# sangminwoo/SVOL

Measured on AMD Instinct MI355X. Metric: frames/sec (fwd+matcher+bwd), T=32·P=196·d=256, higher is better.
Workload: dtype bf16

## Files before the change

### svol_amd/blocks.py

```python
from __future__ import annotations

import ctypes
import math
import os
import weakref

import torch

from . import _lib, layers, ops, params, wgrad

ENABLED = os.environ.get('SVOL_NO_BLOCKS') is None
GATE_SCORES_FUSE = os.environ.get('SVOL_GATE_SCORES_FUSE') is not None
VH, QS, QC = 0, 1, 2
_F32, _BF16 = 0, 1
_ESZ = {torch.float32: 4, torch.bfloat16: 2, torch.float16: 2}
_SLOTS = {}


def _slots(block):
    m = _SLOTS.get(block)
    if m is None:
        names = _lib.lib().svol_block_slot_names(block).decode().rstrip(',').split(',')
        m = _SLOTS[block] = {n: i for i, n in enumerate(names)}
    return m
# ... 283 lines not shown
class _DqPrezero:
    __slots__ = ('bufs', 'side', 'ev_prep', 'clean_ev', 'clean', 'nxt')

    def __init__(self, dev, wsb):
        self.bufs = [torch.empty((_align(wsb, 1 << 20),), dtype=torch.uint8, device=dev) for _ in range(2)]
        self.side = torch.cuda.Stream(device=dev)
        self.ev_prep = torch.cuda.Event()
        self.clean_ev = [torch.cuda.Event(), torch.cuda.Event()]
        for e_ in [self.ev_prep] + self.clean_ev:
            e_.record()
        self.clean = [False, False]
        self.nxt = 0

    def bind(self, tbl):
        i = self.nxt
        tbl.set('ATTN_WS', self.bufs[i].data_ptr())
        tbl.set('EV_CLEAN_IN', self.clean_ev[i].cuda_event if self.clean[i] else None)
        tbl.set('EV_PREP', self.ev_prep.cuda_event)
        tbl.set('ATTN_WS_NEXT', self.bufs[1 - i].data_ptr())
        tbl.set('ZERO_STREAM', self.side.cuda_stream)
        tbl.set('EV_CLEAN_OUT', self.clean_ev[1 - i].cuda_event)
        self.clean[i] = False

    def advance(self, tbl):
        i = self.nxt
        self.clean[1 - i] = True
        self.nxt = 1 - i
        for n_ in ('EV_CLEAN_IN', 'EV_PREP', 'ATTN_WS_NEXT', 'ZERO_STREAM', 'EV_CLEAN_OUT'):
            tbl.set(n_, None)


def _dq_prezero(dev, B, H, L, dh, dt, wsb):
    if not DQ_PREZERO or dt == torch.float32 or torch.cuda.is_current_stream_capturing():
        return None
    key = (dev, ops._stream(), B, H, L, dh, dt, wsb)
    st = _DQ_PREZERO.get(key)
    if st is None:
        img = _lib.lib().svol_attn_bwd_sp_image_bytes(B, H, L, L, dh, wsb, ops._DT[dt])
        st = _DQ_PREZERO[key] = _DqPrezero(dev, wsb) if img > 0 else False
    return st or None


def _vh_fwd_layout(B, L, D, H, F, e):
    M = B * L
    return [('Y1', M * D * e), ('Y1POS', M * D * e), ('A', M * 4), ('MEAN1', M * 4), ('RSTD1', M * 4), ('GATE_WS', B * H * (L + 2) * 4),
            ('QKV', M * 3 * D * e), ('O', M * D * e), ('LSE', B * H * L * 4), ('S2', M * D * 4), ('Y2', M * D * e), ('MEAN2', M * 4),
            ('RSTD2', M * 4), ('PRE', M * F * e), ('HID', M * F * e), ('S3', M * D * 4), ('MEAN3', M * 4), ('RSTD3', M * 4),
            ('M32', M * D * 4), ('M', M * D * e), ('MPOS', M * D * e)]


def _vh_bwd_layout(B, L, D, H, F, e):
    M = B * L
    return [('DS32_3', M * D * 4), ('DS3', M * D * e), ('DPRE', M * F * e), ('DY2', M * D * e), ('DS32_2', M * D * 4), ('G2D', M * D * e),
            ('DO', M * D * e), ('DQKV', M * 3 * D * e), ('DELTA', 3 * B * H * L * 4), ('DXQP', M * D * e), ('DXQ', M * D * e),
            ('GATE_WS2', (B * L + B * H) * 4), ('DX32', M * D * 4)]


def _attn_events(tbl, ev):
    tbl.set('EV_A0', ev[0].cuda_event if ev else None)
    tbl.set('EV_A1', ev[1].cuda_event if ev else None)


class VideoHalfFn(torch.autograd.Function):

    @staticmethod
    def forward(ctx, pl, x32, pos, u, u_next, sc_in, *params):
        B, L, D = x32.shape
        layer = pl.layer()
        H, F = layer.nhead, layer.mlp1.fc1.weight.shape[0]
        dt = pl.dt
        e = _ESZ[dt]
        dev = x32.device
        M = B * L
        x2, pos2, u = _c(x32.reshape(M, D)), _c(pos.reshape(M, D)), _c(u)
        assert x2.dtype == torch.float32 and pos2.dtype == dt and u.dtype == torch.float32
        wsb = ops.attn_ws_bytes(dt, B, H, L, L, D // H)
        lay = _open(ctx, pl, VH, (B, L, D, H, F, dt), _dims(B, L, 0, D, H, F, dt, dt, wsb), len(params), dev,
                    lambda: _vh_fwd_layout(B, L, D, H, F, e),
                    lambda: [('Y1_32', M * D * 4), ('Y2_32', M * D * 4), ('ATTN_WS', max(wsb, 16))], X32=x2, POS=pos2, U=u)
        tbl = ctx.tbl
        if sc_in is not None:
            assert sc_in.dtype == torch.float32 and sc_in.numel() == B * H * (L + 2) and sc_in.is_contiguous()
            tbl.set('GATE_WS', sc_in.data_ptr())
            tbl.set('GATE_PRE', sc_in.data_ptr())
        if u_next is not None:
            u_next = u_next.contiguous()
            assert u_next.dtype == torch.float32 and u_next.shape == u.shape and L % 4 == 0
            sc_next = torch.empty((B * H * (L + 2),), dtype=torch.float32, device=dev)
            tbl.set('U_NEXT', u_next.data_ptr())
            tbl.set('GATE_WS_NEXT', sc_next.data_ptr())
        else:
            sc_next = torch.empty((0,), dtype=torch.float32, device=dev)
        ctx.big = wgrad.attn_forward(B * H * L * L)
        _attn_events(tbl, _maybe_events('attn_fwd', (B, H, L, L, D // H)))
        _call('svol_video_half_fwd', ctx)
        _attn_events(tbl, None)
        tbl.set('U_NEXT', None)
        tbl.set('GATE_WS_NEXT', None)
        ctx.shape = (B, L, D, H, F)
        ctx.sc_in = sc_in
        ctx.save_for_backward(x2, pos2, u)
        ctx.mark_non_differentiable(sc_next)
        return (lay.view(ctx.arena, 'M32', torch.float32, (B, L, D)), lay.view(ctx.arena, 'M', dt, (B, L, D)),
                lay.view(ctx.arena, 'MPOS', dt, (B, L, D)), sc_next)

    @staticmethod
    def backward(ctx, dm32, dm, dmpos, _dsc=None):
# ... 49 lines not shown

class QuerySelfFn(torch.autograd.Function):

    @staticmethod
    def forward(ctx, pl, o32, o, opos, qpos, *params):
        B, N, D = o.shape
        H, qdt = pl.layer().nhead, pl.qdt
        e, R = _ESZ[qdt], B * N
        o32_, o_, opos_, qpos_ = _c(o32), _c(o), _c(opos), _c(qpos)
        assert o32_.dtype == torch.float32 and o_.dtype == qdt and opos_.dtype == qdt and qpos_.dtype == qdt
        wsb = ops.attn_ws_bytes(qdt, B, H, N, N, D // H)
        lay = _open(ctx, pl, QS, (B, N, D, H, qdt), _dims(B, 0, N, D, H, 0, qdt, qdt, wsb), len(params), o.device,
                    lambda: [('QKV', R * 3 * D * e), ('OA', R * D * e), ('LSE', B * H * N * 4), ('S4', R * D * 4), ('MEAN4', R * 4),
                             ('RSTD4', R * 4), ('Y32', R * D * 4), ('Y', R * D * e), ('YPOS', R * D * e)],
                    lambda: [('ATTN_WS', max(wsb, 16))], O32=o32_, O=o_, OPOS=opos_, QPOS=qpos_)
        _call('svol_query_self_fwd', ctx)
        ctx.shape = (B, N, D, H)
        ctx.save_for_backward(o32_, o_, opos_, qpos)
        return (lay.view(ctx.arena, 'Y32', torch.float32, (B, N, D)), lay.view(ctx.arena, 'Y', qdt, (B, N, D)),
                lay.view(ctx.arena, 'YPOS', qdt, (B, N, D)))

    @staticmethod
    def backward(ctx, dy32, dy, dypos):
        if dy32 is None and dy is None and dypos is None:
            return _no_grads(ctx, 5)
        B, N, D, H = ctx.shape
        o32_, o_, opos_, qpos = ctx.saved_tensors
        qdt = ctx.pl.qdt
        e, R = _ESZ[qdt], B * N
        gq = _qpos_target(ctx, qpos, ctx.needs_input_grad[4], N, D)
        lay, tmp, bufs, gs = _open_bwd(ctx, o_.device, lambda: [('G', R * D * e), ('DOA', R * D * e), ('DQKV', R * 3 * D * e),
                                                               ('DELTA', 3 * B * H * N * 4), ('DO32', R * D * 4), ('DXQ', R * D * e),
                                                               ('DXQP', R * D * e)], DY32=dy32, DY=dy, DYPOS=dypos)
        _call('svol_query_self_bwd', ctx)
        pg = _close_bwd(ctx, 'svol_query_self_wgrad', bufs, [ctx.arena, tmp, o_, opos_], 5)
        v = lambda n_, dt_: lay.view(tmp, n_, dt_, (B, N, D))
        return (None, v('DO32', torch.float32), v('DXQ', qdt), v('DXQP', qdt), _qpos_grad(gq, qdt)) + pg


def query_self(layer, out, qpos, dt, qdt):
    pl = plan(layer, QS, dt, qdt)
    o32, o, opos = out
    return QuerySelfFn.apply(pl, o32, o, opos, qpos, *pl.inputs(o32, o, opos))


def _qc_fwd_layout(B, N, L, D, H, F, e, qe):
    R, M = B * N, B * L
    return [('Q', R * D * qe), ('QC', R * D * e), ('KV', M * 2 * D * e), ('OA', R * D * e), ('OAQ', R * D * qe), ('LSE', B * H * N * 4),
            ('S5', R * D * 4), ('Y5_32', R * D * 4), ('Y5', R * D * qe), ('MEAN5', R * 4), ('RSTD5', R * 4), ('PRE', R * F * qe),
            ('HID', R * F * qe), ('S6', R * D * 4), ('MEAN6', R * 4), ('RSTD6', R * 4), ('Y32', R * D * 4), ('Y', R * D * qe),
            ('YPOS', R * D * qe)]


def _qc_bwd_layout(B, N, L, D, H, F, e, qe):
    R, M = B * N, B * L
    return [('DS32_6', R * D * 4), ('DS6', R * D * qe), ('DPRE', R * F * qe), ('DY5', R * D * qe), ('G5D', R * D * qe), ('DOAQ', R * D * qe),
            ('DOA', R * D * e), ('DQC', R * D * e), ('DQ', R * D * qe), ('DKV', M * 2 * D * e), ('DELTA', 3 * B * H * N * 4),
            ('DO32', R * D * 4), ('DXQP', R * D * qe), ('DMPOS', M * D * e), ('DMV', M * D * e)]


class QueryCrossFn(torch.autograd.Function):

    @staticmethod
    def forward(ctx, pl, o32, o, opos, mv, mpos, kbias, qpos, *params):
        B, N, D = o.shape
        L = mv.shape[1]
        layer = pl.layer()
        H, F = layer.nhead, layer.mlp2.fc1.weight.shape[0]
        dt, qdt = pl.dt, pl.qdt
        e, qe = _ESZ[dt], _ESZ[qdt]
        o32_, o_, opos_, mv_, mpos_, kb_, qpos_ = _c(o32), _c(o), _c(opos), _c(mv), _c(mpos), _c(kbias), _c(qpos)
        assert o32_.dtype == torch.float32 and o_.dtype == qdt and opos_.dtype == qdt and qpos_.dtype == qdt
        assert mv_.dtype == dt and mpos_.dtype == dt and kb_.dtype == torch.float32
        wsb = ops.attn_ws_bytes(dt, B, H, N, L, D // H)
        lay = _open(ctx, pl, QC, (B, N, L, D, H, F, dt, qdt), _dims(B, L, N, D, H, F, dt, qdt, wsb), len(params), o.device,
                    lambda: _qc_fwd_layout(B, N, L, D, H, F, e, qe), lambda: [('ATTN_WS', max(wsb, 16))],
                    O32=o32_, O=o_, OPOS=opos_, MV=mv_, MPOS=mpos_, KBIAS=kb_, QPOS=qpos_)
        _call('svol_query_cross_fwd', ctx)
        ctx.shape = (B, N, L, D, H, F)
        ctx.save_for_backward(o32_, o_, opos_, mv_, mpos_, kb_, qpos)
        return (lay.view(ctx.arena, 'Y32', torch.float32, (B, N, D)), lay.view(ctx.arena, 'Y', qdt, (B, N, D)),
                lay.view(ctx.arena, 'YPOS', qdt, (B, N, D)))

    @staticmethod
    def backward(ctx, dy32, dy, dypos):
        if dy32 is None and dy is None and dypos is None:
            return _no_grads(ctx, 8)
        B, N, L, D, H, F = ctx.shape
        o32_, o_, opos_, mv_, mpos_, kb_, qpos = ctx.saved_tensors
        dt, qdt = ctx.pl.dt, ctx.pl.qdt
        gq = _qpos_target(ctx, qpos, ctx.needs_input_grad[7], N, D)
        lay, tmp, bufs, gs = _open_bwd(ctx, o_.device, lambda: _qc_bwd_layout(B, N, L, D, H, F, _ESZ[dt], _ESZ[qdt]),
                                       DY32=dy32, DY=dy, DYPOS=dypos)
        _call('svol_query_cross_bwd', ctx)
        pg = _close_bwd(ctx, 'svol_query_cross_wgrad', bufs, [ctx.arena, tmp, opos_, mv_, mpos_], 8)
        vq = lambda n_, dt_: lay.view(tmp, n_, dt_, (B, N, D))
        vm = lambda n_: lay.view(tmp, n_, dt, (B, L, D))
        return (None, vq('DO32', torch.float32), None, vq('DXQP', qdt), vm('DMV'), vm('DMPOS'), None, _qpos_grad(gq, qdt)) + pg


def query_cross(layer, out, mv, mpos, kbias, qpos, dt, qdt):
    pl = plan(layer, QC, dt, qdt)
    o32, o, opos = out
    return QueryCrossFn.apply(pl, o32, o, opos, mv, mpos, kbias, qpos, *pl.inputs(o32, opos, mv, mpos))


def trace_dump() -> str:
    buf = ctypes.create_string_buffer(1 << 20)
    _lib.check(_lib.lib().svol_block_trace_dump(buf, len(buf)), 'svol_block_trace_dump')
    return buf.value.decode()
```

### svol_amd/csrc/blocks.hip

```cpp
#include <math.h>
#include <stdio.h>
#include <stdlib.h>
#include <string.h>

#include <map>
#include <mutex>
#include <string>
#include <vector>

#include "common.h"

namespace {

const bool kTrace = getenv("SVOL_BLOCK_TRACE") != nullptr;
struct TraceRec { const char* prog; const char* site; hipEvent_t e0, e1; };
std::mutex g_trace_mu;
std::vector<TraceRec> g_trace_log;
struct Trace {
    const char* prog;
    hipStream_t s;
    hipEvent_t last = nullptr;
    Trace* prev;
    static thread_local Trace* cur;
    Trace(const char* prog_, void* s_) : prog(prog_), s(static_cast<hipStream_t>(s_)), prev(cur) {
// ... 151 lines not shown
        RUN(nt(P(Y1), D, at(P(W_IN), 2 * D * D, dt), D, at(P(QKV), 2 * D, dt), 3 * D, f32(P(B_IN)) + 2 * D, nullptr, M, D, D, dt, s));
    record(P(EV_A0), s);
    RUN(svol_attn_fwd(P(QKV), 3 * D, at(P(QKV), D, dt), 3 * D, at(P(QKV), 2 * D, dt), 3 * D, P(O), D, f32(P(LSE)), nullptr, d.B, d.H, d.L,
                      d.L, dh, attn_scale(dh), attn_premul(dh, dt), P(ATTN_WS), d.ws_bytes, dt, s));
    record(P(EV_A1), s);
    RUN(nt_res(P(O), D, P(W_O), D, P(S2), P(B_O), P(Y1_32), M, D, D, dt, s));
    RUN(svol_layernorm_fwd(P(S2), xf, f32(P(G2)), f32(P(BT2)), f32(P(Y2_32)), P(Y2), nullptr, nullptr, 0, f32(P(MEAN2)), f32(P(RSTD2)), M,
                           D, 0.f, 0, nullptr, dt, s));
    RUN(svol_gemm_nt(P(Y2), D, nullptr, 0, P(W_FC1), D, P(HID), F, f32(P(B_FC1)), nullptr, SVOL_ACT_GELU_D, P(PRE), F, nullptr, 0, 0, M, F, D, dt, s));
    RUN(nt_res(P(HID), F, P(W_FC2), F, P(S3), P(B_FC2), P(Y2_32), M, D, F, dt, s));
    if (P(U_NEXT) && P(GATE_WS_NEXT))
        RUN(svol_layernorm_gate_scores_fwd(f32(P(S3)), f32(P(G3)), f32(P(BT3)), f32(P(M32)), P(M), P(MPOS), P(POS), f32(P(MEAN3)),
                                           f32(P(RSTD3)), f32(P(U_NEXT)), f32(P(GATE_WS_NEXT)), d.B, d.L, D, d.H, dt, s));
    else
        RUN(svol_layernorm_fwd(P(S3), xf, f32(P(G3)), f32(P(BT3)), f32(P(M32)), P(M), P(MPOS), P(POS), M, f32(P(MEAN3)), f32(P(RSTD3)), M, D,
                               0.f, 0, nullptr, dt, s));
    return SVOL_OK;
}

int svol_video_half_bwd(const int64_t* dims, void* const* p, int phase, void* s) {
    if (!dims || !p || phase < 0 || phase > 2) return SVOL_E_INVALID;
    Trace tr_(phase == 2 ? "video_half_bwd.2" : "video_half_bwd.1", s);
    const Dims d(dims);
    if (!d.ok() || d.L <= 0 || d.F <= 0) return SVOL_E_INVALID;
    const int64_t M = d.B * d.L, D = d.D, F = d.F, dh = D / d.H;
    const int dt = d.dt, xf = dt != SVOL_F32;
    if (phase != 2) {
        RUN(svol_layernorm_bwd(f32(P(DM32)), P(DM), P(DMPOS), P(S3), xf, f32(P(G3)), f32(P(MEAN3)), f32(P(RSTD3)), f32(P(DS32_3)), P(DS3),
                               f32(P(DG3)), f32(P(DBT3)), f32(P(DB_FC2)), M, D, 0.f, 0, nullptr, dt, s));
        RUN(svol_gemm_nt_dact(P(DS3), D, P(W_FC2_T), D, P(DPRE), F, P(PRE), F, SVOL_ACT_GELU_D, f32(P(DB_FC1)), M, F, D, dt, s));
        RUN(nt(P(DPRE), F, P(W_FC1_T), F, P(DY2), D, nullptr, nullptr, M, D, F, dt, s));
        RUN(svol_layernorm_bwd(f32(P(DS32_3)), P(DY2), nullptr, P(S2), xf, f32(P(G2)), f32(P(MEAN2)), f32(P(RSTD2)), f32(P(DS32_2)), P(G2D),
                               f32(P(DG2)), f32(P(DBT2)), f32(P(DB_O)), M, D, 0.f, 0, nullptr, dt, s));
        RUN(nt(P(G2D), D, P(W_O_T), D, P(DO), D, nullptr, nullptr, M, D, D, dt, s));
    }
    if (phase != 1) {
        int aflags = 0;
        if (P(EV_CLEAN_IN)) {
            if (hipStreamWaitEvent(static_cast<hipStream_t>(s), static_cast<hipEvent_t>(P(EV_CLEAN_IN)), 0) != hipSuccess) return SVOL_E_LAUNCH;
            aflags = SVOL_ATTN_DQ_PREZEROED;
        }
        record(P(EV_A0), s);
        RUN(svol_attn_bwd_ex(P(QKV), 3 * D, at(P(QKV), D, dt), 3 * D, at(P(QKV), 2 * D, dt), 3 * D, P(O), D, P(DO), D, f32(P(LSE)),
                             f32(P(DELTA)), nullptr, P(DQKV), 3 * D, at(P(DQKV), D, dt), 3 * D, at(P(DQKV), 2 * D, dt), 3 * D, d.B, d.H, d.L,
                             d.L, dh, attn_scale(dh), attn_premul(dh, dt), P(ATTN_WS), d.ws_bytes, dt, aflags, P(EV_PREP), s));
        record(P(EV_A1), s);
        if (P(ATTN_WS_NEXT) && P(ZERO_STREAM) && P(EV_PREP) && P(EV_CLEAN_OUT)) {
            hipStream_t zs = static_cast<hipStream_t>(P(ZERO_STREAM));
            if (hipStreamWaitEvent(zs, static_cast<hipEvent_t>(P(EV_PREP)), 0) != hipSuccess) return SVOL_E_LAUNCH;
            const int zrc = svol_attn_bwd_zero_ws(P(ATTN_WS_NEXT), d.ws_bytes, d.B, d.H, d.L, d.L, dh, dt, zs);
            if (zrc) return zrc;
            record(P(EV_CLEAN_OUT), zs);
        }
        RUN(nt(P(DQKV), 3 * D, P(W_IN_T), 3 * D, P(DXQP), D, nullptr, nullptr, M, D, 2 * D, dt, s));
        RUN(nt(at(P(DQKV), 2 * D, dt), 3 * D, at(P(W_IN_T), 2 * D, dt), 3 * D, P(DXQ), D, nullptr, nullptr, M, D, D, dt, s));
        RUN(svol_gate_bwd(f32(P(DS32_2)), P(DXQ), P(DXQP), f32(P(X32)), P(POS), f32(P(U)), f32(P(G1)), f32(P(A)), f32(P(MEAN1)),
                          f32(P(RSTD1)), f32(P(GATE_WS)), f32(P(GATE_WS2)), f32(P(DX32)), f32(P(DU)), f32(P(DG1)), f32(P(DBT1)), d.B, d.L,
                          D, d.H, dt, s));
    }
    return SVOL_OK;
}

int svol_video_half_wgrad_part(const int64_t* dims, void* const* p, int part, void* s) {
    if (!dims || !p || part < 0 || part > 2) return SVOL_E_INVALID;
    Trace tr_(part == 1 ? "video_half_wgrad.1" : part == 2 ? "video_half_wgrad.2" : "video_half_wgrad", s);
    const Dims d(dims);
    if (!d.ok()) return SVOL_E_INVALID;
    const int64_t M = d.B * d.L, D = d.D, F = d.F;
    const int dt = d.dt;
    const svol_tn_problem pr[5] = {
        {P(DS3), D, P(HID), F, f32(P(DW_FC2)), F, nullptr, M, D, F},
        {P(DPRE), F, P(Y2), D, f32(P(DW_FC1)), D, nullptr, M, F, D},
        {P(G2D), D, P(O), D, f32(P(DW_O)), D, nullptr, M, D, D},
        {P(DQKV), 3 * D, P(Y1POS), D, f32(P(DW_IN)), D, f32(P(DB_IN)), M, 2 * D, D},
        {at(P(DQKV), 2 * D, dt), 3 * D, P(Y1), D, f32(P(DW_IN)) + 2 * D * D, D, f32(P(DB_IN)) + 2 * D, M, D, D}};
    if (part == 1) RUN(svol_gemm_tn_grouped(pr, 3, dt, s));
    else if (part == 2) RUN(svol_gemm_tn_grouped(pr + 3, 2, dt, s));
    else RUN(svol_gemm_tn_grouped(pr, 5, dt, s));
    return SVOL_OK;
}

int svol_video_half_wgrad(const int64_t* dims, void* const* p, void* s) { return svol_video_half_wgrad_part(dims, p, 0, s); }
#undef P

int svol_query_self_fwd(const int64_t* dims, void* const* p, void* s) {
    if (!dims || !p) return SVOL_E_INVALID;
    Trace tr_("query_self_fwd", s);
    const Dims d(dims);
    if (!d.ok() || d.N <= 0) return SVOL_E_INVALID;
    const int64_t R = d.B * d.N, D = d.D, dh = D / d.H;
    const int qdt = d.qdt, xf = qdt != SVOL_F32;
#define P(n) p[SVOL_QS_##n]
    RUN(nt(P(OPOS), D, P(W_IN), D, P(QKV), 3 * D, P(B_IN), P(QSCALE), R, 2 * D, D, qdt, s));
    if (P(WV_HILO))
        RUN(svol_gemm_nt_split(P(O), D, P(WV_HILO), 2 * D, at(P(QKV), 2 * D, qdt), 3 * D, f32(P(B_IN)) + 2 * D, R, D, D, s));
    else
        RUN(nt(P(O), D, at(P(W_IN), 2 * D * D, qdt), D, at(P(QKV), 2 * D, qdt), 3 * D, f32(P(B_IN)) + 2 * D, nullptr, R, D, D, qdt, s));
    RUN(svol_attn_fwd(P(QKV), 3 * D, at(P(QKV), D, qdt), 3 * D, at(P(QKV), 2 * D, qdt), 3 * D, P(OA), D, f32(P(LSE)), nullptr, d.B, d.H,
                      d.N, d.N, dh, attn_scale(dh), attn_premul(dh, qdt), P(ATTN_WS), d.ws_bytes, qdt, s));
    RUN(nt_res(P(OA), D, P(W_O), D, P(S4), P(B_O), P(O32), R, D, D, qdt, s));
    RUN(svol_layernorm_fwd(P(S4), xf, f32(P(G4)), f32(P(BT4)), f32(P(Y32)), P(Y), P(YPOS), P(QPOS), d.N, f32(P(MEAN4)), f32(P(RSTD4)), R, D,
                           0.f, 0, nullptr, qdt, s));
    return SVOL_OK;
}

int svol_query_self_bwd(const int64_t* dims, void* const* p, void* s) {
    if (!dims || !p) return SVOL_E_INVALID;
    Trace tr_("query_self_bwd", s);
    const Dims d(dims);
// ... 41 lines not shown
    if (mixed) {
        RUN(nt(P(OPOS), D, P(W_INQ), D, P(Q), D, P(B_IN), P(QSCALE), R, D, D, qdt, s));
        RUN(svol_cast(P(Q), qdt, P(QC), dt, R * D, s));
    } else {
        RUN(nt(P(OPOS), D, P(W_KV), D, P(QC), D, P(B_IN), P(QSCALE), R, D, D, dt, s));
    }
    RUN(nt(P(MPOS), D, at(P(W_KV), D * D, dt), D, P(KV), 2 * D, f32(P(B_IN)) + D, nullptr, M, D, D, dt, s));
    if (P(WV_HILO))
        RUN(svol_gemm_nt_split(P(MV), D, P(WV_HILO), 2 * D, at(P(KV), D, dt), 2 * D, f32(P(B_IN)) + 2 * D, M, D, D, s));
    else
        RUN(nt(P(MV), D, at(P(W_KV), 2 * D * D, dt), D, at(P(KV), D, dt), 2 * D, f32(P(B_IN)) + 2 * D, nullptr, M, D, D, dt, s));
    RUN(svol_attn_fwd(P(QC), D, P(KV), 2 * D, at(P(KV), D, dt), 2 * D, P(OA), D, f32(P(LSE)), f32(P(KBIAS)), d.B, d.H, d.N, d.L, dh,
                      attn_scale(dh), attn_premul(dh, dt), P(ATTN_WS), d.ws_bytes, dt, s));
    const void* oq = P(OA);
    if (mixed) {
        RUN(svol_cast(P(OA), dt, P(OAQ), qdt, R * D, s));
        oq = P(OAQ);
    }
    RUN(nt_res(oq, D, P(W_O), D, P(S5), P(B_O), P(O32), R, D, D, qdt, s));
    RUN(svol_layernorm_fwd(P(S5), xf, f32(P(G5)), f32(P(BT5)), f32(P(Y5_32)), P(Y5), nullptr, nullptr, 0, f32(P(MEAN5)), f32(P(RSTD5)), R,
                           D, 0.f, 0, nullptr, qdt, s));
    RUN(svol_gemm_nt(P(Y5), D, nullptr, 0, P(W_FC1), D, P(HID), F, f32(P(B_FC1)), nullptr, SVOL_ACT_GELU, P(PRE), F, nullptr, 0, 0, R, F, D,
                     qdt, s));
    RUN(nt_res(P(HID), F, P(W_FC2), F, P(S6), P(B_FC2), P(Y5_32), R, D, F, qdt, s));
    RUN(svol_layernorm_fwd(P(S6), xf, f32(P(G6)), f32(P(BT6)), f32(P(Y32)), P(Y), P(YPOS), P(QPOS), d.N, f32(P(MEAN6)), f32(P(RSTD6)), R, D,
                           0.f, 0, nullptr, qdt, s));
    return SVOL_OK;
}

int svol_query_cross_bwd(const int64_t* dims, void* const* p, void* s) {
    if (!dims || !p) return SVOL_E_INVALID;
    Trace tr_("query_cross_bwd", s);
    const Dims d(dims);
    if (!d.ok() || d.N <= 0 || d.L <= 0 || d.F <= 0) return SVOL_E_INVALID;
    const int64_t R = d.B * d.N, M = d.B * d.L, D = d.D, F = d.F, dh = D / d.H;
    const int dt = d.dt, qdt = d.qdt, xf = qdt != SVOL_F32;
    const bool mixed = qdt != dt;
    RUN(svol_layernorm_bwd(f32(P(DY32)), P(DY), P(DYPOS), P(S6), xf, f32(P(G6)), f32(P(MEAN6)), f32(P(RSTD6)), f32(P(DS32_6)), P(DS6),
                           f32(P(DG6)), f32(P(DBT6)), f32(P(DB_FC2)), R, D, 0.f, 0, nullptr, qdt, s));
    if (P(DQPOS) && P(DYPOS)) RUN(svol_colsum(P(DYPOS), d.N * D, f32(P(DQPOS)), d.B, d.N * D, qdt, s));
    RUN(svol_gemm_nt_dact(P(DS6), D, P(W_FC2_T), D, P(DPRE), F, P(PRE), F, SVOL_ACT_GELU, f32(P(DB_FC1)), R, F, D, qdt, s));
    RUN(nt(P(DPRE), F, P(W_FC1_T), F, P(DY5), D, nullptr, nullptr, R, D, F, qdt, s));
    RUN(svol_layernorm_bwd(f32(P(DS32_6)), P(DY5), nullptr, P(S5), xf, f32(P(G5)), f32(P(MEAN5)), f32(P(RSTD5)), f32(P(DO32)), P(G5D),
                           f32(P(DG5)), f32(P(DBT5)), f32(P(DB_O)), R, D, 0.f, 0, nullptr, qdt, s));
    RUN(nt(P(G5D), D, P(W_O_T), D, P(DOAQ), D, nullptr, nullptr, R, D, D, qdt, s));
    const void* d_o = P(DOAQ);
    if (mixed) {
        RUN(svol_cast(P(DOAQ), qdt, P(DOA), dt, R * D, s));
        d_o = P(DOA);
    }
    RUN(svol_attn_bwd(P(QC), D, P(KV), 2 * D, at(P(KV), D, dt), 2 * D, P(OA), D, d_o, D, f32(P(LSE)), f32(P(DELTA)), f32(P(KBIAS)), P(DQC), D,
                      P(DKV), 2 * D, at(P(DKV), D, dt), 2 * D, d.B, d.H, d.N, d.L, dh, attn_scale(dh), attn_premul(dh, dt), P(ATTN_WS),
                      d.ws_bytes, dt, s));
    RUN(nt(P(DKV), 2 * D, at(P(W_KV_T), D, dt), 3 * D, P(DMPOS), D, nullptr, nullptr, M, D, D, dt, s));
    RUN(nt(at(P(DKV), D, dt), 2 * D, at(P(W_KV_T), 2 * D, dt), 3 * D, P(DMV), D, nullptr, nullptr, M, D, D, dt, s));
    const void* dq = P(DQC);
    if (mixed) {
        RUN(svol_cast(P(DQC), dt, P(DQ), qdt, R * D, s));
        dq = P(DQ);
    }
    RUN(nt(dq, D, mixed ? P(W_INQ_T) : P(W_KV_T), 3 * D, P(DXQP), D, nullptr, nullptr, R, D, D, qdt, s));
    return SVOL_OK;
}

int svol_query_cross_wgrad(const int64_t* dims, void* const* p, void* s) {
    if (!dims || !p) return SVOL_E_INVALID;
    Trace tr_("query_cross_wgrad", s);
    const Dims d(dims);
    if (!d.ok()) return SVOL_E_INVALID;
    const int64_t R = d.B * d.N, M = d.B * d.L, D = d.D, F = d.F;
    const int dt = d.dt, qdt = d.qdt;
    const bool mixed = qdt != dt;
    const svol_tn_problem pv[2] = {
        {P(DKV), 2 * D, P(MPOS), D, f32(P(DW_IN)) + D * D, D, f32(P(DB_IN)) + D, M, D, D},
        {at(P(DKV), D, dt), 2 * D, P(MV), D, f32(P(DW_IN)) + 2 * D * D, D, f32(P(DB_IN)) + 2 * D, M, D, D}};
    RUN(svol_gemm_tn_grouped(pv, 2, dt, s));
    const svol_tn_problem pq[4] = {
        {P(DS6), D, P(HID), F, f32(P(DW_FC2)), F, nullptr, R, D, F},
        {P(DPRE), F, P(Y5), D, f32(P(DW_FC1)), D, nullptr, R, F, D},
        {P(G5D), D, mixed ? P(OAQ) : P(OA), D, f32(P(DW_O)), D, nullptr, R, D, D},
        {mixed ? P(DQ) : P(DQC), D, P(OPOS), D, f32(P(DW_IN)), D, f32(P(DB_IN)), R, D, D}};
    RUN(svol_gemm_tn_grouped(pq, 4, qdt, s));
    return SVOL_OK;
#undef P
}

}
```

### svol_amd/csrc/gemm_n256_bf16.hip

```cpp
#include <type_traits>

#include "gemm_call.h"

namespace {

struct N256Args {
    const h16_t* A; const h16_t* W; void* C;
    const float* bias; const float* res;
    int64_t lda, ldw, ldc, ldr;
    int M, K, act, nrt;
    int kwt;
};

typedef __attribute__((address_space(3))) void* lds_void_ptr;

constexpr int BM = 128, BN = 256, BK = 32, STG = 3;
constexpr int A_ST = BM * BK * 2;
constexpr int W_ST = BN * BK * 2;
constexpr int SLOT = A_ST + W_ST;

__device__ __forceinline__ int slot32(int row, int ch) { return ch ^ ((0x78 >> (2 * ((row >> 2) & 3))) & 3); }
__device__ __forceinline__ int wcol(int nt, int i) { return (nt >> 1) * 32 + (i >> 2) * 8 + (nt & 1) * 4 + (i & 3); }

template <int N> __device__ __forceinline__ void n256_wait_vm() { asm volatile("s_waitcnt vmcnt(%0)" ::"n"(N) : "memory"); }

template <int OFF>
__device__ __forceinline__ void read_frags(uint4 (&af)[4], uint4 (&wf)[8], const unsigned (&aa)[4], const unsigned (&wa)[8]) {
    asm volatile(
        "ds_read_b128 %0, %12 offset:%c24\n\t"
        "ds_read_b128 %1, %13 offset:%c24\n\t"
        "ds_read_b128 %2, %14 offset:%c24\n\t"
        "ds_read_b128 %3, %15 offset:%c24\n\t"
        "ds_read_b128 %4, %16 offset:%c25\n\t"
        "ds_read_b128 %5, %17 offset:%c25\n\t"
        "ds_read_b128 %6, %18 offset:%c25\n\t"
        "ds_read_b128 %7, %19 offset:%c25\n\t"
        "ds_read_b128 %8, %20 offset:%c25\n\t"
        "ds_read_b128 %9, %21 offset:%c25\n\t"
        "ds_read_b128 %10, %22 offset:%c25\n\t"
        "ds_read_b128 %11, %23 offset:%c25\n\t"
        "s_waitcnt lgkmcnt(0)"
        : "=&v"(af[0]), "=&v"(af[1]), "=&v"(af[2]), "=&v"(af[3]), "=&v"(wf[0]), "=&v"(wf[1]), "=&v"(wf[2]), "=&v"(wf[3]),
          "=&v"(wf[4]), "=&v"(wf[5]), "=&v"(wf[6]), "=&v"(wf[7])
        : "v"(aa[0]), "v"(aa[1]), "v"(aa[2]), "v"(aa[3]), "v"(wa[0]), "v"(wa[1]), "v"(wa[2]), "v"(wa[3]), "v"(wa[4]), "v"(wa[5]),
          "v"(wa[6]), "v"(wa[7]), "n"(OFF), "n"(OFF + A_ST)
        : "memory");
}

template <bool OUT_F32>
__device__ __forceinline__ void gemm_n256_body(const N256Args& p) {
    __shared__ __attribute__((aligned(1024))) char smem[STG * SLOT];
    const int tid = threadIdx.x, lane = tid & 63;
    const int wave = __builtin_amdgcn_readfirstlane(tid >> 6);
    const int wm = wave >> 1, wn = wave & 1;
    const int fr = lane & 15, fq = lane >> 4;
    const int rt = blockIdx.x % p.nrt, cg = blockIdx.x / p.nrt;
    const int bm = rt * BM;
    if (bm >= p.M) return;
    const int rows = min(BM, p.M - bm);
    const int bn = cg * BN;

    const __amdgpu_buffer_rsrc_t rA = __builtin_amdgcn_make_buffer_rsrc(
        (void*)(p.A + (int64_t)bm * p.lda), 0, (int)((((int64_t)rows - 1) * p.lda + p.kwt * BK) * 2), 0x00020000);
    const __amdgpu_buffer_rsrc_t rW =
        __builtin_amdgcn_make_buffer_rsrc((void*)(p.W + (int64_t)bn * p.ldw), 0, (int)((((int64_t)BN - 1) * p.ldw + p.K) * 2), 0x00020000);
    int voffA[2], voffW[4];
#pragma unroll
    for (int j = 0; j < 2; ++j) {
        const int row = (wave * 2 + j) * 16 + (lane >> 2);
        voffA[j] = (int)(((int64_t)row * p.lda + slot32(row, lane & 3) * 8) * 2);
    }
#pragma unroll
    for (int j = 0; j < 4; ++j) {
        const int rho = (wave * 4 + j) * 16 + (lane >> 2);
        const int n = (rho >> 7) * 128 + wcol((rho & 127) >> 4, rho & 15);
        voffW[j] = (int)(((int64_t)n * p.ldw + slot32(rho, lane & 3) * 8) * 2);
    }
    auto issue = [&](int slot, int kt) {
        char* sl = smem + slot * SLOT;
        const int so = kt * BK * 2;
        const int soA = (kt >= p.kwt ? kt - p.kwt : kt) * BK * 2;
#pragma unroll
        for (int j = 0; j < 2; ++j)
            __builtin_amdgcn_raw_ptr_buffer_load_lds(rA, (lds_void_ptr)(sl + (wave * 2 + j) * 1024), 16, voffA[j], soA, 0, 0);
#pragma unroll
        for (int j = 0; j < 4; ++j)
            __builtin_amdgcn_raw_ptr_buffer_load_lds(rW, (lds_void_ptr)(sl + A_ST + (wave * 4 + j) * 1024), 16, voffW[j], so, 0, 0);
    };

    const unsigned lds0 = (unsigned)(size_t)(lds_void_ptr)smem;
    unsigned aa[4], wa[8];
#pragma unroll
    for (int mt = 0; mt < 4; ++mt) {
        const int row = wm * 64 + mt * 16 + fr;
        aa[mt] = lds0 + (unsigned)(row * 64 + (slot32(row, fq) << 4));
    }
#pragma unroll
    for (int nt = 0; nt < 8; ++nt) {
        const int rho = wn * 128 + nt * 16 + fr;
        wa[nt] = lds0 + (unsigned)(rho * 64 + (slot32(rho, fq) << 4));
    }

    f32x4 acc[8][4];
#pragma unroll
    for (int i = 0; i < 8; ++i)
#pragma unroll
        for (int j = 0; j < 4; ++j) acc[i][j] = f32x4{0.f, 0.f, 0.f, 0.f};

    const int nk = p.K / BK;
    issue(0, 0);
    if (nk > 1) issue(1, 1);
    auto step = [&](auto slot_tag, int kt) {
        constexpr int S = decltype(slot_tag)::value;
        if (kt + 1 < nk) n256_wait_vm<6>(); else n256_wait_vm<0>();
        __builtin_amdgcn_s_barrier();
        if (kt + 2 < nk) issue((S + 2) % STG, kt + 2);
        uint4 af[4], wf[8];
        read_frags<S * SLOT>(af, wf, aa, wa);
#pragma unroll
        for (int nt = 0; nt < 8; ++nt)
#pragma unroll
            for (int mt = 0; mt < 4; ++mt)
                acc[nt][mt] = SVOL_MFMA_16x16x32_H16(__builtin_bit_cast(h16x8, wf[nt]),
                                                                      __builtin_bit_cast(h16x8, af[mt]), acc[nt][mt], 0, 0, 0);
    };
    int kt = 0;
    for (; kt + 3 <= nk; kt += 3) {
        step(std::integral_constant<int, 0>{}, kt);
        step(std::integral_constant<int, 1>{}, kt + 1);
        step(std::integral_constant<int, 2>{}, kt + 2);
    }
    if (kt < nk) step(std::integral_constant<int, 0>{}, kt++);
    if (kt < nk) step(std::integral_constant<int, 1>{}, kt++);

#pragma unroll
    for (int mt = 0; mt < 4; ++mt) {
        const int m = bm + wm * 64 + mt * 16 + fr;
        if (m >= p.M) continue;
#pragma unroll
        for (int pr = 0; pr < 4; ++pr) {
            const int n0 = bn + wn * 128 + pr * 32 + fq * 8;
            float v[8];
#pragma unroll
            for (int e = 0; e < 8; ++e) v[e] = acc[2 * pr + (e >> 2)][mt][e & 3];
            if (p.bias) {
#pragma unroll
                for (int e = 0; e < 8; ++e) v[e] += p.bias[n0 + e];
            }
            if constexpr (OUT_F32) {
                float* C = reinterpret_cast<float*>(p.C) + (int64_t)m * p.ldc + n0;
                if (p.res) {
                    const float* R = p.res + (int64_t)m * p.ldr + n0;
                    const f32x4 r0 = *reinterpret_cast<const f32x4*>(R), r1 = *reinterpret_cast<const f32x4*>(R + 4);
#pragma unroll
                    for (int e = 0; e < 4; ++e) { v[e] += r0[e]; v[4 + e] += r1[e]; }
                }
                *reinterpret_cast<f32x4*>(C) = f32x4{v[0], v[1], v[2], v[3]};
                *reinterpret_cast<f32x4*>(C + 4) = f32x4{v[4], v[5], v[6], v[7]};
            } else {
                if (act_is_gelu(p.act)) {
#pragma unroll
                    for (int e = 0; e < 8; ++e) v[e] = gelu_fast(v[e]);
                }
                if (p.act == SVOL_ACT_RELU) {
#pragma unroll
                    for (int e = 0; e < 8; ++e) v[e] = fmaxf(v[e], 0.f);
                }
                h16x8 o;
#pragma unroll
                for (int e = 0; e < 8; ++e) o[e] = (h16_t)v[e];
                *reinterpret_cast<h16x8*>(reinterpret_cast<h16_t*>(p.C) + (int64_t)m * p.ldc + n0) = o;
            }
        }
    }
}

__global__ __launch_bounds__(256, 2) void gemm_n256_bf16_f32(N256Args p) { gemm_n256_body<true>(p); }
__global__ __launch_bounds__(256, 2) void gemm_n256_bf16_b16(N256Args p) { gemm_n256_body<false>(p); }

}

static int n256_plan(const GemmCall& c, N256Args& p, dim3& grid) {
    const int64_t M = c.M, N = c.N, K = c.K;
    if (N % BN || K % BK || K < 512 || M < 4096) return SVOL_E_UNSUPPORTED;
    if (c.epi != 0 || c.pre || c.colscale) return SVOL_E_UNSUPPORTED;
    if (c.kwrap != K && (c.kwrap % BK || 2 * c.kwrap != K)) return SVOL_E_UNSUPPORTED;
    if (c.act != SVOL_ACT_NONE && ((c.act != SVOL_ACT_GELU && c.act != SVOL_ACT_RELU) || c.out_f32)) return SVOL_E_UNSUPPORTED;
    if (c.res && !c.out_f32) return SVOL_E_UNSUPPORTED;
    if (c.lda % 8 || c.ldb % 8 || !aligned16(c.A) || !aligned16(c.B) || !aligned16(c.C)) return SVOL_E_UNSUPPORTED;
    if (c.out_f32 ? (c.ldc % 4 || (c.res && (c.ldr % 4 || !aligned16(c.res)))) : (c.ldc % 8 != 0)) return SVOL_E_UNSUPPORTED;
    if ((int64_t)BM * c.lda * 2 >= (1ll << 31) || (int64_t)BN * c.ldb * 2 >= (1ll << 31)) return SVOL_E_UNSUPPORTED;
    const int64_t ncg = N / BN;
    int64_t nrt = (M + BM - 1) / BM;
    if (ncg > 1) nrt = (nrt + 7) / 8 * 8;
    if (nrt * ncg > (1ll << 30)) return SVOL_E_UNSUPPORTED;
    p = N256Args{(const h16_t*)c.A, (const h16_t*)c.B, c.C, c.bias, (const float*)c.res, c.lda, c.ldb, c.ldc, c.ldr, (int)M, (int)K, c.act,
                 (int)nrt, (int)(c.kwrap / BK)};
    grid = dim3((unsigned)(nrt * ncg));
    return SVOL_OK;
}

int svol_gemm_n256_bf16(const GemmCall& c) {
    N256Args p; dim3 grid;
    if (const int rc = n256_plan(c, p, grid)) return rc;
    hipLaunchKernelGGL(c.out_f32 ? gemm_n256_bf16_f32 : gemm_n256_bf16_b16, grid, dim3(256), 0, c.stream, p);
    return hipGetLastError() == hipSuccess ? SVOL_OK : SVOL_E_LAUNCH;
}
```

Baseline: 14790.

## Merge split backward GEMMs and add CU-balanced N256 GEMM variant

In the video-half backward, the two input-projection grad GEMMs (q/k part and v part) become one GEMM with K=3D, and the gate backward reads a single summed gradient. In query-cross backward, when mv and mpos come from the same VideoHalf node, the DMPOS and DMV GEMMs merge into one K=2D GEMM writing DMV only. Separately, the N=256 GEMM gains a 512-thread balanced variant that sizes row tiles to the CU count, so single-column-group launches spread work evenly across CUs instead of leaving a partial last wave. This cuts launches and tail imbalance, but it relies on the gradient sum being mathematically equivalent and on the autograd graph check to pick the merged path.

Measured after the change: 15030 (median of 6 runs). 1.6% higher.

```diff
diff --git a/svol_amd/blocks.py b/svol_amd/blocks.py
--- a/svol_amd/blocks.py
+++ b/svol_amd/blocks.py
@@ -359,7 +359,7 @@
 def _vh_bwd_layout(B, L, D, H, F, e):
     M = B * L
     return [('DS32_3', M * D * 4), ('DS3', M * D * e), ('DPRE', M * F * e), ('DY2', M * D * e), ('DS32_2', M * D * 4), ('G2D', M * D * e),
-            ('DO', M * D * e), ('DQKV', M * 3 * D * e), ('DELTA', 3 * B * H * L * 4), ('DXQP', M * D * e), ('DXQ', M * D * e),
+            ('DO', M * D * e), ('DQKV', M * 3 * D * e), ('DELTA', 3 * B * H * L * 4), ('DXQ', M * D * e),
             ('GATE_WS2', (B * L + B * H) * 4), ('DX32', M * D * 4)]
 
 
@@ -515,17 +515,17 @@
             ('YPOS', R * D * qe)]
 
 
-def _qc_bwd_layout(B, N, L, D, H, F, e, qe):
+def _qc_bwd_layout(B, N, L, D, H, F, e, qe, merged):
     R, M = B * N, B * L
     return [('DS32_6', R * D * 4), ('DS6', R * D * qe), ('DPRE', R * F * qe), ('DY5', R * D * qe), ('G5D', R * D * qe), ('DOAQ', R * D * qe),
             ('DOA', R * D * e), ('DQC', R * D * e), ('DQ', R * D * qe), ('DKV', M * 2 * D * e), ('DELTA', 3 * B * H * N * 4),
-            ('DO32', R * D * 4), ('DXQP', R * D * qe), ('DMPOS', M * D * e), ('DMV', M * D * e)]
+            ('DO32', R * D * 4), ('DXQP', R * D * qe)] + ([] if merged else [('DMPOS', M * D * e)]) + [('DMV', M * D * e)]
 
 
 class QueryCrossFn(torch.autograd.Function):
 
     @staticmethod
-    def forward(ctx, pl, o32, o, opos, mv, mpos, kbias, qpos, *params):
+    def forward(ctx, pl, o32, o, opos, mv, mpos, kbias, qpos, merged, *params):
         B, N, D = o.shape
         L = mv.shape[1]
         layer = pl.layer()
@@ -536,11 +536,12 @@
         assert o32_.dtype == torch.float32 and o_.dtype == qdt and opos_.dtype == qdt and qpos_.dtype == qdt
         assert mv_.dtype == dt and mpos_.dtype == dt and kb_.dtype == torch.float32
         wsb = ops.attn_ws_bytes(dt, B, H, N, L, D // H)
-        lay = _open(ctx, pl, QC, (B, N, L, D, H, F, dt, qdt), _dims(B, L, N, D, H, F, dt, qdt, wsb), len(params), o.device,
+        lay = _open(ctx, pl, QC, (B, N, L, D, H, F, dt, qdt, merged), _dims(B, L, N, D, H, F, dt, qdt, wsb), len(params), o.device,
                     lambda: _qc_fwd_layout(B, N, L, D, H, F, e, qe), lambda: [('ATTN_WS', max(wsb, 16))],
                     O32=o32_, O=o_, OPOS=opos_, MV=mv_, MPOS=mpos_, KBIAS=kb_, QPOS=qpos_)
         _call('svol_query_cross_fwd', ctx)
         ctx.shape = (B, N, L, D, H, F)
+        ctx.merged = merged
         ctx.save_for_backward(o32_, o_, opos_, mv_, mpos_, kb_, qpos)
         return (lay.view(ctx.arena, 'Y32', torch.float32, (B, N, D)), lay.view(ctx.arena, 'Y', qdt, (B, N, D)),
                 lay.view(ctx.arena, 'YPOS', qdt, (B, N, D)))
@@ -548,24 +549,27 @@
     @staticmethod
     def backward(ctx, dy32, dy, dypos):
         if dy32 is None and dy is None and dypos is None:
-            return _no_grads(ctx, 8)
+            return _no_grads(ctx, 9)
         B, N, L, D, H, F = ctx.shape
         o32_, o_, opos_, mv_, mpos_, kb_, qpos = ctx.saved_tensors
         dt, qdt = ctx.pl.dt, ctx.pl.qdt
         gq = _qpos_target(ctx, qpos, ctx.needs_input_grad[7], N, D)
-        lay, tmp, bufs, gs = _open_bwd(ctx, o_.device, lambda: _qc_bwd_layout(B, N, L, D, H, F, _ESZ[dt], _ESZ[qdt]),
+        lay, tmp, bufs, gs = _open_bwd(ctx, o_.device, lambda: _qc_bwd_layout(B, N, L, D, H, F, _ESZ[dt], _ESZ[qdt], ctx.merged),
                                        DY32=dy32, DY=dy, DYPOS=dypos)
         _call('svol_query_cross_bwd', ctx)
-        pg = _close_bwd(ctx, 'svol_query_cross_wgrad', bufs, [ctx.arena, tmp, opos_, mv_, mpos_], 8)
+        pg = _close_bwd(ctx, 'svol_query_cross_wgrad', bufs, [ctx.arena, tmp, opos_, mv_, mpos_], 9)
         vq = lambda n_, dt_: lay.view(tmp, n_, dt_, (B, N, D))
         vm = lambda n_: lay.view(tmp, n_, dt, (B, L, D))
-        return (None, vq('DO32', torch.float32), None, vq('DXQP', qdt), vm('DMV'), vm('DMPOS'), None, _qpos_grad(gq, qdt)) + pg
+        return (None, vq('DO32', torch.float32), None, vq('DXQP', qdt), vm('DMV'), None if ctx.merged else vm('DMPOS'), None,
+                _qpos_grad(gq, qdt), None) + pg
 
 
 def query_cross(layer, out, mv, mpos, kbias, qpos, dt, qdt):
     pl = plan(layer, QC, dt, qdt)
     o32, o, opos = out
-    return QueryCrossFn.apply(pl, o32, o, opos, mv, mpos, kbias, qpos, *pl.inputs(o32, opos, mv, mpos))
+    fn = mv.grad_fn
+    merged = fn is not None and fn is mpos.grad_fn and isinstance(fn, VideoHalfFn._backward_cls)
+    return QueryCrossFn.apply(pl, o32, o, opos, mv, mpos, kbias, qpos, merged, *pl.inputs(o32, opos, mv, mpos))
 
 
 def trace_dump() -> str:
diff --git a/svol_amd/csrc/blocks.hip b/svol_amd/csrc/blocks.hip
--- a/svol_amd/csrc/blocks.hip
+++ b/svol_amd/csrc/blocks.hip
@@ -227,9 +227,8 @@
             if (zrc) return zrc;
             record(P(EV_CLEAN_OUT), zs);
         }
-        RUN(nt(P(DQKV), 3 * D, P(W_IN_T), 3 * D, P(DXQP), D, nullptr, nullptr, M, D, 2 * D, dt, s));
-        RUN(nt(at(P(DQKV), 2 * D, dt), 3 * D, at(P(W_IN_T), 2 * D, dt), 3 * D, P(DXQ), D, nullptr, nullptr, M, D, D, dt, s));
-        RUN(svol_gate_bwd(f32(P(DS32_2)), P(DXQ), P(DXQP), f32(P(X32)), P(POS), f32(P(U)), f32(P(G1)), f32(P(A)), f32(P(MEAN1)),
+        RUN(nt(P(DQKV), 3 * D, P(W_IN_T), 3 * D, P(DXQ), D, nullptr, nullptr, M, D, 3 * D, dt, s));
+        RUN(svol_gate_bwd(f32(P(DS32_2)), P(DXQ), nullptr, f32(P(X32)), P(POS), f32(P(U)), f32(P(G1)), f32(P(A)), f32(P(MEAN1)),
                           f32(P(RSTD1)), f32(P(GATE_WS)), f32(P(GATE_WS2)), f32(P(DX32)), f32(P(DU)), f32(P(DG1)), f32(P(DBT1)), d.B, d.L,
                           D, d.H, dt, s));
     }
@@ -377,8 +376,12 @@
     RUN(svol_attn_bwd(P(QC), D, P(KV), 2 * D, at(P(KV), D, dt), 2 * D, P(OA), D, d_o, D, f32(P(LSE)), f32(P(DELTA)), f32(P(KBIAS)), P(DQC), D,
                       P(DKV), 2 * D, at(P(DKV), D, dt), 2 * D, d.B, d.H, d.N, d.L, dh, attn_scale(dh), attn_premul(dh, dt), P(ATTN_WS),
                       d.ws_bytes, dt, s));
-    RUN(nt(P(DKV), 2 * D, at(P(W_KV_T), D, dt), 3 * D, P(DMPOS), D, nullptr, nullptr, M, D, D, dt, s));
-    RUN(nt(at(P(DKV), D, dt), 2 * D, at(P(W_KV_T), 2 * D, dt), 3 * D, P(DMV), D, nullptr, nullptr, M, D, D, dt, s));
+    if (P(DMPOS)) {
+        RUN(nt(P(DKV), 2 * D, at(P(W_KV_T), D, dt), 3 * D, P(DMPOS), D, nullptr, nullptr, M, D, D, dt, s));
+        RUN(nt(at(P(DKV), D, dt), 2 * D, at(P(W_KV_T), 2 * D, dt), 3 * D, P(DMV), D, nullptr, nullptr, M, D, D, dt, s));
+    } else {
+        RUN(nt(P(DKV), 2 * D, at(P(W_KV_T), D, dt), 3 * D, P(DMV), D, nullptr, nullptr, M, D, 2 * D, dt, s));
+    }
     const void* dq = P(DQC);
     if (mixed) {
         RUN(svol_cast(P(DQC), dt, P(DQ), qdt, R * D, s));
diff --git a/svol_amd/csrc/gemm_n256_bf16.hip b/svol_amd/csrc/gemm_n256_bf16.hip
--- a/svol_amd/csrc/gemm_n256_bf16.hip
+++ b/svol_amd/csrc/gemm_n256_bf16.hip
@@ -9,22 +9,37 @@
     const float* bias; const float* res;
     int64_t lda, ldw, ldc, ldr;
     int M, K, act, nrt;
+    int rpw;
     int kwt;
 };
 
 typedef __attribute__((address_space(3))) void* lds_void_ptr;
 
-constexpr int BM = 128, BN = 256, BK = 32, STG = 3;
-constexpr int A_ST = BM * BK * 2;
+constexpr int BM = 128, BN = 256, BK = 32, BAL_BM = 256;
 constexpr int W_ST = BN * BK * 2;
-constexpr int SLOT = A_ST + W_ST;
+constexpr int BAL_STG = 3;
+template <bool BAL> struct Ring {
+    static constexpr int bm = BAL ? BAL_BM : BM, waves = bm / 32, stg = BAL ? BAL_STG : 3;
+    static constexpr int a_st = bm * BK * 2, slot = a_st + W_ST, bytes = stg * slot;
+    static constexpr int wpw = 16 / waves;
+    static constexpr int pieces = 2 + wpw;
+    static constexpr int w_base = BAL ? stg * a_st : 0;
+    static constexpr int offa(int s) { return BAL ? s * a_st : s * slot; }
+    static constexpr int offw(int s) { return BAL ? s * W_ST : s * slot + a_st; }
+    static_assert(offa(stg - 1) < 65536 && offw(stg - 1) < 65536 && bytes <= 160 * 1024, "ring does not fit");
+};
 
 __device__ __forceinline__ int slot32(int row, int ch) { return ch ^ ((0x78 >> (2 * ((row >> 2) & 3))) & 3); }
 __device__ __forceinline__ int wcol(int nt, int i) { return (nt >> 1) * 32 + (i >> 2) * 8 + (nt & 1) * 4 + (i & 3); }
 
 template <int N> __device__ __forceinline__ void n256_wait_vm() { asm volatile("s_waitcnt vmcnt(%0)" ::"n"(N) : "memory"); }
-
-template <int OFF>
+template <int PIECES, int F> __device__ __forceinline__ void n256_wait_slabs(int fly) {
+    if constexpr (F == 0) n256_wait_vm<0>();
+    else if (fly >= F) n256_wait_vm<PIECES * F>();
+    else n256_wait_slabs<PIECES, F - 1>(fly);
+}
+
+template <int OFFA, int OFFW>
 __device__ __forceinline__ void read_frags(uint4 (&af)[4], uint4 (&wf)[8], const unsigned (&aa)[4], const unsigned (&wa)[8]) {
     asm volatile(
         "ds_read_b128 %0, %12 offset:%c24\n\t"
@@ -43,62 +58,77 @@
         : "=&v"(af[0]), "=&v"(af[1]), "=&v"(af[2]), "=&v"(af[3]), "=&v"(wf[0]), "=&v"(wf[1]), "=&v"(wf[2]), "=&v"(wf[3]),
           "=&v"(wf[4]), "=&v"(wf[5]), "=&v"(wf[6]), "=&v"(wf[7])
         : "v"(aa[0]), "v"(aa[1]), "v"(aa[2]), "v"(aa[3]), "v"(wa[0]), "v"(wa[1]), "v"(wa[2]), "v"(wa[3]), "v"(wa[4]), "v"(wa[5]),
-          "v"(wa[6]), "v"(wa[7]), "n"(OFF), "n"(OFF + A_ST)
+          "v"(wa[6]), "v"(wa[7]), "n"(OFFA), "n"(OFFW)
         : "memory");
 }
 
-template <bool OUT_F32>
+template <int S, int STG, class F> __device__ __forceinline__ void ring_pass(F& step, int kt) {
+    if constexpr (S < STG) { step(std::integral_constant<int, S>{}, kt + S); ring_pass<S + 1, STG>(step, kt); }
+}
+template <int S, int STG, class F> __device__ __forceinline__ void ring_tail(F& step, int kt, int nk) {
+    if constexpr (S < STG - 1) {
+        if (kt < nk) { step(std::integral_constant<int, S>{}, kt); ring_tail<S + 1, STG>(step, kt + 1, nk); }
+    }
+}
+
+template <bool OUT_F32, bool BAL>
 __device__ __forceinline__ void gemm_n256_body(const N256Args& p) {
-    __shared__ __attribute__((aligned(1024))) char smem[STG * SLOT];
+    using R = Ring<BAL>;
+    constexpr int STG = R::stg;
+    __shared__ __attribute__((aligned(1024))) char smem[R::bytes];
     const int tid = threadIdx.x, lane = tid & 63;
     const int wave = __builtin_amdgcn_readfirstlane(tid >> 6);
     const int wm = wave >> 1, wn = wave & 1;
     const int fr = lane & 15, fq = lane >> 4;
-    const int rt = blockIdx.x % p.nrt, cg = blockIdx.x / p.nrt;
-    const int bm = rt * BM;
+    const int rt = BAL ? blockIdx.x : blockIdx.x % p.nrt, cg = BAL ? 0 : blockIdx.x / p.nrt;
+    const int bm = rt * (BAL ? p.rpw : BM);
     if (bm >= p.M) return;
-    const int rows = min(BM, p.M - bm);
+    const int rows = min(BAL ? p.rpw : BM, p.M - bm);
     const int bn = cg * BN;
+    const int ntile = (rows + 15) >> 4;
+    const int t0 = BAL ? (wm * ntile) >> 2 : wm * 4;
+    const int cnt = BAL ? (((wm + 1) * ntile) >> 2) - t0 : 4;
 
     const __amdgpu_buffer_rsrc_t rA = __builtin_amdgcn_make_buffer_rsrc(
         (void*)(p.A + (int64_t)bm * p.lda), 0, (int)((((int64_t)rows - 1) * p.lda + p.kwt * BK) * 2), 0x00020000);
     const __amdgpu_buffer_rsrc_t rW =
         __builtin_amdgcn_make_buffer_rsrc((void*)(p.W + (int64_t)bn * p.ldw), 0, (int)((((int64_t)BN - 1) * p.ldw + p.K) * 2), 0x00020000);
-    int voffA[2], voffW[4];
+    int voffA[2], voffW[R::wpw];
 #pragma unroll
     for (int j = 0; j < 2; ++j) {
         const int row = (wave * 2 + j) * 16 + (lane >> 2);
         voffA[j] = (int)(((int64_t)row * p.lda + slot32(row, lane & 3) * 8) * 2);
     }
 #pragma unroll
-    for (int j = 0; j < 4; ++j) {
-        const int rho = (wave * 4 + j) * 16 + (lane >> 2);
+    for (int j = 0; j < R::wpw; ++j) {
+        const int rho = (wave * R::wpw + j) * 16 + (lane >> 2);
         const int n = (rho >> 7) * 128 + wcol((rho & 127) >> 4, rho & 15);
         voffW[j] = (int)(((int64_t)n * p.ldw + slot32(rho, lane & 3) * 8) * 2);
     }
     auto issue = [&](int slot, int kt) {
-        char* sl = smem + slot * SLOT;
+        char* slA = smem + (BAL ? slot * R::a_st : slot * R::slot);
+        char* slW = smem + (BAL ? R::w_base + slot * W_ST : slot * R::slot + R::a_st);
         const int so = kt * BK * 2;
         const int soA = (kt >= p.kwt ? kt - p.kwt : kt) * BK * 2;
 #pragma unroll
         for (int j = 0; j < 2; ++j)
-            __builtin_amdgcn_raw_ptr_buffer_load_lds(rA, (lds_void_ptr)(sl + (wave * 2 + j) * 1024), 16, voffA[j], soA, 0, 0);
-#pragma unroll
-        for (int j = 0; j < 4; ++j)
-            __builtin_amdgcn_raw_ptr_buffer_load_lds(rW, (lds_void_ptr)(sl + A_ST + (wave * 4 + j) * 1024), 16, voffW[j], so, 0, 0);
+            __builtin_amdgcn_raw_ptr_buffer_load_lds(rA, (lds_void_ptr)(slA + (wave * 2 + j) * 1024), 16, voffA[j], soA, 0, 0);
+#pragma unroll
+        for (int j = 0; j < R::wpw; ++j)
+            __builtin_amdgcn_raw_ptr_buffer_load_lds(rW, (lds_void_ptr)(slW + (wave * R::wpw + j) * 1024), 16, voffW[j], so, 0, 0);
     };
 
     const unsigned lds0 = (unsigned)(size_t)(lds_void_ptr)smem;
     unsigned aa[4], wa[8];
 #pragma unroll
     for (int mt = 0; mt < 4; ++mt) {
-        const int row = wm * 64 + mt * 16 + fr;
+        const int row = (t0 + mt) * 16 + fr;
         aa[mt] = lds0 + (unsigned)(row * 64 + (slot32(row, fq) << 4));
     }
 #pragma unroll
     for (int nt = 0; nt < 8; ++nt) {
         const int rho = wn * 128 + nt * 16 + fr;
-        wa[nt] = lds0 + (unsigned)(rho * 64 + (slot32(rho, fq) << 4));
+        wa[nt] = lds0 + (unsigned)(R::w_base + rho * 64 + (slot32(rho, fq) << 4));
     }
 
     f32x4 acc[8][4];
@@ -108,35 +138,43 @@
         for (int j = 0; j < 4; ++j) acc[i][j] = f32x4{0.f, 0.f, 0.f, 0.f};
 
     const int nk = p.K / BK;
-    issue(0, 0);
-    if (nk > 1) issue(1, 1);
+#pragma unroll
+    for (int s = 0; s < STG - 1; ++s)
+        if (s < nk) issue(s, s);
     auto step = [&](auto slot_tag, int kt) {
         constexpr int S = decltype(slot_tag)::value;
-        if (kt + 1 < nk) n256_wait_vm<6>(); else n256_wait_vm<0>();
+        n256_wait_slabs<R::pieces, STG - 2>(nk - 1 - kt);
         __builtin_amdgcn_s_barrier();
-        if (kt + 2 < nk) issue((S + 2) % STG, kt + 2);
+        if (kt + STG - 1 < nk) issue((S + STG - 1) % STG, kt + STG - 1);
         uint4 af[4], wf[8];
-        read_frags<S * SLOT>(af, wf, aa, wa);
-#pragma unroll
-        for (int nt = 0; nt < 8; ++nt)
+        read_frags<R::offa(S), R::offw(S)>(af, wf, aa, wa);
+        if constexpr (BAL) {
 #pragma unroll
             for (int mt = 0; mt < 4; ++mt)
-                acc[nt][mt] = SVOL_MFMA_16x16x32_H16(__builtin_bit_cast(h16x8, wf[nt]),
-                                                                      __builtin_bit_cast(h16x8, af[mt]), acc[nt][mt], 0, 0, 0);
+                if (mt < cnt) {
+#pragma unroll
+                    for (int nt = 0; nt < 8; ++nt)
+                        acc[nt][mt] = SVOL_MFMA_16x16x32_H16(__builtin_bit_cast(h16x8, wf[nt]),
+                                                                              __builtin_bit_cast(h16x8, af[mt]), acc[nt][mt], 0, 0, 0);
+                }
+        } else {
+#pragma unroll
+            for (int nt = 0; nt < 8; ++nt)
+#pragma unroll
+                for (int mt = 0; mt < 4; ++mt)
+                    acc[nt][mt] = SVOL_MFMA_16x16x32_H16(__builtin_bit_cast(h16x8, wf[nt]),
+                                                                          __builtin_bit_cast(h16x8, af[mt]), acc[nt][mt], 0, 0, 0);
+        }
     };
     int kt = 0;
-    for (; kt + 3 <= nk; kt += 3) {
-        step(std::integral_constant<int, 0>{}, kt);
-        step(std::integral_constant<int, 1>{}, kt + 1);
-        step(std::integral_constant<int, 2>{}, kt + 2);
-    }
-    if (kt < nk) step(std::integral_constant<int, 0>{}, kt++);
-    if (kt < nk) step(std::integral_constant<int, 1>{}, kt++);
+    for (; kt + STG <= nk; kt += STG) ring_pass<0, STG>(step, kt);
+    ring_tail<0, STG>(step, kt, nk);
 
 #pragma unroll
     for (int mt = 0; mt < 4; ++mt) {
-        const int m = bm + wm * 64 + mt * 16 + fr;
-        if (m >= p.M) continue;
+        const int lr = (t0 + mt) * 16 + fr;
+        const int m = bm + lr;
+        if (mt >= cnt || lr >= rows) continue;
 #pragma unroll
         for (int pr = 0; pr < 4; ++pr) {
             const int n0 = bn + wn * 128 + pr * 32 + fq * 8;
@@ -175,12 +213,23 @@
     }
 }
 
-__global__ __launch_bounds__(256, 2) void gemm_n256_bf16_f32(N256Args p) { gemm_n256_body<true>(p); }
-__global__ __launch_bounds__(256, 2) void gemm_n256_bf16_b16(N256Args p) { gemm_n256_body<false>(p); }
-
-}
-
-static int n256_plan(const GemmCall& c, N256Args& p, dim3& grid) {
+__global__ __launch_bounds__(256, 2) void gemm_n256_bf16_f32(N256Args p) { gemm_n256_body<true, false>(p); }
+__global__ __launch_bounds__(256, 2) void gemm_n256_bf16_b16(N256Args p) { gemm_n256_body<false, false>(p); }
+__global__ __launch_bounds__(512, 2) void gemm_n256_bal_bf16_f32(N256Args p) { gemm_n256_body<true, true>(p); }
+__global__ __launch_bounds__(512, 2) void gemm_n256_bal_bf16_b16(N256Args p) { gemm_n256_body<false, true>(p); }
+
+}
+
+static int n256_cus() {
+    static const int n = [] {
+        int dev = 0, cus = 0;
+        if (hipGetDevice(&dev) != hipSuccess || hipDeviceGetAttribute(&cus, hipDeviceAttributeMultiprocessorCount, dev) != hipSuccess) return 0;
+        return cus;
+    }();
+    return n;
+}
+
+static int n256_plan(const GemmCall& c, N256Args& p, dim3& grid, bool& bal) {
     const int64_t M = c.M, N = c.N, K = c.K;
     if (N % BN || K % BK || K < 512 || M < 4096) return SVOL_E_UNSUPPORTED;
     if (c.epi != 0 || c.pre || c.colscale) return SVOL_E_UNSUPPORTED;
@@ -190,19 +239,24 @@
     if (c.lda % 8 || c.ldb % 8 || !aligned16(c.A) || !aligned16(c.B) || !aligned16(c.C)) return SVOL_E_UNSUPPORTED;
     if (c.out_f32 ? (c.ldc % 4 || (c.res && (c.ldr % 4 || !aligned16(c.res)))) : (c.ldc % 8 != 0)) return SVOL_E_UNSUPPORTED;
     if ((int64_t)BM * c.lda * 2 >= (1ll << 31) || (int64_t)BN * c.ldb * 2 >= (1ll << 31)) return SVOL_E_UNSUPPORTED;
-    const int64_t ncg = N / BN;
-    int64_t nrt = (M + BM - 1) / BM;
-    if (ncg > 1) nrt = (nrt + 7) / 8 * 8;
+    const int64_t ncg = N / BN, cus = n256_cus();
+    bal = ncg == 1 && cus > 0 && M > BM * cus && (int64_t)BAL_BM * c.lda * 2 < (1ll << 31);
+    int64_t nrt = (M + BM - 1) / BM, rpw = 0;
+    if (bal) {
+        nrt = cus * ((M + BAL_BM * cus - 1) / (BAL_BM * cus));
+        rpw = (M + nrt - 1) / nrt;
+    } else if (ncg > 1) nrt = (nrt + 7) / 8 * 8;
     if (nrt * ncg > (1ll << 30)) return SVOL_E_UNSUPPORTED;
     p = N256Args{(const h16_t*)c.A, (const h16_t*)c.B, c.C, c.bias, (const float*)c.res, c.lda, c.ldb, c.ldc, c.ldr, (int)M, (int)K, c.act,
-                 (int)nrt, (int)(c.kwrap / BK)};
+                 (int)nrt, (int)rpw, (int)(c.kwrap / BK)};
     grid = dim3((unsigned)(nrt * ncg));
     return SVOL_OK;
 }
 
 int svol_gemm_n256_bf16(const GemmCall& c) {
-    N256Args p; dim3 grid;
-    if (const int rc = n256_plan(c, p, grid)) return rc;
-    hipLaunchKernelGGL(c.out_f32 ? gemm_n256_bf16_f32 : gemm_n256_bf16_b16, grid, dim3(256), 0, c.stream, p);
+    N256Args p; dim3 grid; bool bal;
+    if (const int rc = n256_plan(c, p, grid, bal)) return rc;
+    if (bal) hipLaunchKernelGGL(c.out_f32 ? gemm_n256_bal_bf16_f32 : gemm_n256_bal_bf16_b16, grid, dim3(512), 0, c.stream, p);
+    else hipLaunchKernelGGL(c.out_f32 ? gemm_n256_bf16_f32 : gemm_n256_bf16_b16, grid, dim3(256), 0, c.stream, p);
     return hipGetLastError() == hipSuccess ? SVOL_OK : SVOL_E_LAUNCH;
 }
```
